# sdrobert/pydrobert-speech

Hardware: AMD Instinct MI355X
Metric: frames/s (whole node) + HBM-roofline %, 40-mel fbank 16kHz 25/10ms (higher is better)
Workload: dtype f32

## Files before the change

pydrobert-speech_amd/csrc/fft_inlane.h:

```cpp
#pragma once
#include <hip/hip_runtime.h>

#include <type_traits>

#include "twiddle_consts.h"

#define PDS_HD __host__ __device__ __forceinline__

#ifndef PDS_FMA_BUTTERFLY
#define PDS_FMA_BUTTERFLY 1
#endif

namespace pds {
namespace inl {

template <int I>
using Int = std::integral_constant<int, I>;

template <int B, int E, typename F>
PDS_HD void static_for(F &&f) {
  if constexpr (B < E) {
    f(Int<B>{});
    static_for<B + 1, E>(f);
  }
// ... 54 lines not shown
        yi[k] = si;
        yr[k + H] = fmaf(2.0f, er[k], -sr);
        yi[k + H] = fmaf(2.0f, ei[k], -si);
        return;
#endif
      }
      float tr, ti;
      mul_tw<N, k>(qr[k], qi[k], tr, ti);
      yr[k] = er[k] + tr;
      yi[k] = ei[k] + ti;
      yr[k + H] = er[k] - tr;
      yi[k + H] = ei[k] - ti;
    });
  }
};

template <int IS>
struct CFFT<1, IS> {
  static PDS_HD void run(const float *xr, const float *xi, float *yr, float *yi) {
    yr[0] = xr[0];
    yi[0] = xi[0];
  }
};

template <int IS>
struct CFFT<2, IS> {
  static PDS_HD void run(const float *xr, const float *xi, float *yr, float *yi) {
    const float ar = xr[0], ai = xi[0], br = xr[IS], bi = xi[IS];
    yr[0] = ar + br;
    yi[0] = ai + bi;
    yr[1] = ar - br;
    yi[1] = ai - bi;
  }
};

template <int IS>
struct CFFT<4, IS> {
  static PDS_HD void run(const float *xr, const float *xi, float *yr, float *yi) {
    const float ar = xr[0] + xr[2 * IS], ai = xi[0] + xi[2 * IS];
    const float br = xr[0] - xr[2 * IS], bi = xi[0] - xi[2 * IS];
    const float cr = xr[IS] + xr[3 * IS], ci = xi[IS] + xi[3 * IS];
    const float dr = xr[IS] - xr[3 * IS], di = xi[IS] - xi[3 * IS];
    yr[0] = ar + cr;
    yi[0] = ai + ci;
    yr[2] = ar - cr;
    yi[2] = ai - ci;
    yr[1] = br + di;
    yi[1] = bi - dr;
    yr[3] = br - di;
    yi[3] = bi + dr;
  }
};

template <int M>
PDS_HD void rdft_scaled(const float *a, float &even_sum, float &odd_sum, float *Ar, float *Ai) {
  constexpr int H = M / 2;
  float zr[H], zi[H];
  CFFT<H, 2>::run(a, a + 1, zr, zi);
  even_sum = zr[0];
  odd_sum = zi[0];
  if constexpr (H >= 2) {
    Ar[H / 2] = zr[H / 2];
    Ai[H / 2] = -zi[H / 2];
  }
  static_for<1, H / 2>([&](auto kk) {
    constexpr int k = decltype(kk)::value;
    const float sr = zr[k] + zr[H - k], si = zi[k] - zi[H - k];
    const float dr = zr[k] - zr[H - k], di = zi[k] + zi[H - k];
    constexpr float wr = Tw<M, k>::re, wi = Tw<M, k>::im;
#if PDS_FMA_BUTTERFLY
    const float ar = fmaf(wr, di, fmaf(wi, dr, sr));
    const float ai = fmaf(wi, di, fmaf(-wr, dr, si));
    Ar[k] = ar;
    Ai[k] = ai;
    Ar[H - k] = fmaf(2.0f, sr, -ar);
    Ai[H - k] = fmaf(-2.0f, si, ai);
#else
    const float tr = wr * di + wi * dr;
    const float ti = wi * di - wr * dr;
    Ar[k] = sr + tr;
    Ai[k] = si + ti;
    Ar[H - k] = sr - tr;
    Ai[H - k] = ti - si;
#endif
  });
}

template <int M, int IS>
struct RDIT {
  static PDS_HD void run(const float *x, float &r0, float &rh, float *Ar, float *Ai) {
    constexpr int H = M / 2, Q = M / 4;
    float e0, eh, o0, oh;
    float Er[Q > 1 ? Q : 1], Ei[Q > 1 ? Q : 1], Or[Q > 1 ? Q : 1], Oi[Q > 1 ? Q : 1];
    RDIT<H, 2 * IS>::run(x, e0, eh, Er, Ei);
    RDIT<H, 2 * IS>::run(x + IS, o0, oh, Or, Oi);
    r0 = e0 + o0;
    rh = e0 - o0;
    Ar[Q] = eh;
    Ai[Q] = -oh;
    static_for<1, Q>([&](auto kk) {
      constexpr int k = decltype(kk)::value;
      constexpr float c = Tw<M, k>::re, s = Tw<M, k>::im;
      const float ar = fmaf(Or[k], c, fmaf(-s, Oi[k], Er[k]));
      const float ai = fmaf(Or[k], s, fmaf(c, Oi[k], Ei[k]));
      Ar[k] = ar;
      Ai[k] = ai;
// ... 322 lines not shown
```

pydrobert-speech_amd/csrc/pds_internal.h:

```cpp
#pragma once
#include <hip/hip_runtime.h>
#include <stdint.h>

#include <exception>
#include <new>
#include <string>

#include "../../include/pds_amd.h"

namespace pds {

void set_error(const std::string &msg);
int32_t hip_fail(hipError_t err, const char *what);

#define PDS_HIP(call)                                       \
  do {                                                      \
    hipError_t _e = (call);                                 \
    if (_e != hipSuccess) return pds::hip_fail(_e, #call);  \
  } while (0)

struct FastTables {
  int kind = 0;
  int n1 = 0, n2 = 0;
  int rows = 0;
  int num_cus = 0;
  float *d_window = nullptr;
  float *d_twiddle = nullptr;
  float *d_tw_special = nullptr;
  float *d_win_half = nullptr;
  float *d_tw_seed = nullptr;
  float *d_ell_w = nullptr;
  int32_t *d_ell_meta = nullptr;
  int32_t *d_ell_len = nullptr;
  int32_t *d_ell_woff = nullptr;
  int ell_wfloats = 0, ell_slots = 0;
  float *d_seg_w = nullptr;
  int32_t *d_seg_meta = nullptr;
  int seg_rounds = 0, seg_len = 0, seg_wfloats = 0, seg_meta_ints = 0;
  float *d_rs_w = nullptr;
  int32_t *d_rs_meta = nullptr;
  int rs_rounds = 0, rs_len = 0, rs_wfloats = 0;
  float *d_rsn_w = nullptr;
  int32_t *d_rsn_meta = nullptr;
  int rsn_rounds = 0, rsn_len = 0, rsn_wfloats = 0;
  int rs_eslot = -1;
  float *d_ms_w = nullptr;
  int32_t *d_ms_meta = nullptr;
  int ms_rounds = 0, ms_len = 0, ms_wfloats = 0, ms_meta_ints = 0, ms_slots = 0;
  long ms_reads = 0;
  int walk = 0;
  long rs_reads = 0, rs_cost = 0, ell_reads = 0, seg_reads = 0;
  float *d_mf_tab = nullptr;
  int mf_rows = 0;
};

}

struct pds_stft_plan {
  pds_stft_desc d;
  int device = 0;
  int num_bins = 0;
  float *d_window_f32 = nullptr;
  double *d_window_f64 = nullptr;
  int32_t *d_row_ptr = nullptr;
  int32_t *d_col = nullptr;
  float *d_val_f32 = nullptr;
  double *d_val_f64 = nullptr;
  float2 *d_tw_f32 = nullptr;
  double2 *d_tw_f64 = nullptr;
  pds::FastTables fast;
};

namespace pds {
struct SiFftTables {
  int blocks = 0;
  bool big = false;
  float2 *d_spectra = nullptr;
  float2 *d_twiddle = nullptr;
  float2 *d_twiddle2k = nullptr;
  int num_cus = 0;
// ... 112 lines not shown
```

pydrobert-speech_amd/csrc/stft_fast.hip:

```cpp
#include "stft_wave_launch.h"

namespace pds {

#if PDS_STAMPS
unsigned long long *g_stamp_buf = nullptr;
extern "C" __attribute__((visibility("default"))) void pds_debug_set_stamp_buffer(unsigned long long *d_buf) {
  g_stamp_buf = d_buf;
}
#endif

extern "C" __attribute__((visibility("default"))) int32_t pds_build_experiments(void) { return PDS_EXPERIMENTS ? 1 : 0; }

bool fast_has_f64in(const pds_stft_plan *plan) { return plan->fast.kind && fast_f64in_kind(plan->fast.kind); }

bool fast_has_fused_cmvn(const pds_stft_plan *plan) {
  const FastTables &ft = plan->fast;
  return ft.kind && ft.n2 == 16 && ((ft.n1 == 64 && ft.walk != 0) || (ft.n1 == 32 && (ft.walk == 1 || ft.walk == 3)));
}

bool fast_has_fused_deltas(const pds_stft_plan *plan) {
  const FastTables &ft = plan->fast;
  return ft.kind && fast_deltas_kind(ft.kind) && ft.rsn_rounds >= 1 && ft.rsn_rounds <= 2 &&
         (!plan->d.include_energy || ft.rs_eslot >= 0);
}
// ... 43 lines not shown
#include "stft_geoms.def"
#endif
#undef PDS_GEOM
  set_error("stft_batch: no fused kernel for this plan");
  return PDS_ERR_INVALID;
}

int32_t fast_tables_create(pds_stft_plan *plan, const double *window, const int32_t *row_ptr,
                           const int32_t *col, const double *val) {
  FastTables &ft = plan->fast;
  ft.kind = 0;
  const pds_stft_desc &d = plan->d;
  int n1 = 0, n2 = 0;
  switch (d.dft_size) {
    case 128: n1 = 16; n2 = 8; break;
    case 256: n1 = 32; n2 = 8; break;
    case 512: n1 = 32; n2 = 16; break;
    case 1024: {
      const char *geom = PDS_EXPERIMENTS ? std::getenv("PDS_N1024_GEOM") : nullptr;
      const bool wide = geom && std::strcmp(geom, "32x32") == 0;
      n1 = wide ? 32 : 64;
      n2 = wide ? 32 : 16;
      break;
    }
    case 2048: n1 = 64; n2 = 32; break;
    case 4096: n1 = 64; n2 = 64; break;
    case 160: n1 = 20; n2 = 8; break;
    case 200: n1 = 25; n2 = 8; break;
    case 240: n1 = 30; n2 = 8; break;
    case 320: n1 = 20; n2 = 16; break;
    case 400: n1 = 25; n2 = 16; break;
    case 480: n1 = 30; n2 = 16; break;
    case 640: n1 = 20; n2 = 32; break;
    case 800: n1 = 25; n2 = 32; break;
    case 960: n1 = 30; n2 = 32; break;
    default: return PDS_OK;
  }
  const bool pow2 = (n1 & (n1 - 1)) == 0;
  if (!pow2 && d.frame_length != d.dft_size) return PDS_OK;
  const char *off = std::getenv("PDS_STFT_GENERIC");
  if (off && off[0] == '1') return PDS_OK;
  if (d.frame_length > d.dft_size || d.frame_length <= d.dft_size / 2) return PDS_OK;
  if (d.frame_shift >= (1 << 22)) return PDS_OK;
  if (d.use_log && !((float)d.log_floor >= 1.17549435e-38f)) return PDS_OK;
  if (d.num_filts > 32767) return PDS_OK;
  const int N = d.dft_size, H1 = n1 / 2, cols = (n1 - 1) / 2 + 1;
  std::vector<float> win((size_t)n1 * n2, 0.0f);
  for (int r = 0; r < n2; ++r)
    for (int k = 0; k < n1; ++k) {
      const int idx = n2 * k + r;
      if (idx < d.frame_length) win[(size_t)r * n1 + k] = (float)window[idx];
    }
  std::vector<float> tw((size_t)n2 * cols * 2, 0.0f);
  for (int r = 0; r < n2; ++r)
    for (int k1 = 1; k1 < cols; ++k1) {
      const double ang = -2.0 * M_PI * (double)((r * k1) % N) / (double)N;
      const double scale = (!pow2 || PDS_RDFT_DIT) ? 1.0 : (2 * k1 == H1) ? 1.0 : 0.5;
      tw[((size_t)r * cols + k1) * 2 + 0] = (float)(scale * std::cos(ang));
      tw[((size_t)r * cols + k1) * 2 + 1] = (float)(scale * std::sin(ang));
    }
  std::vector<int32_t> order(d.num_filts);
  for (int f = 0; f < d.num_filts; ++f) order[f] = f;
  auto span = [&](int f) {
    return row_ptr[f + 1] > row_ptr[f] ? col[row_ptr[f + 1] - 1] - (col[row_ptr[f]] & ~3) + 1 : 0;
  };
  std::stable_sort(order.begin(), order.end(), [&](int x, int y) { return span(x) > span(y); });
  const int slots = (d.num_filts + n2 - 1) / n2;
  const int pstr = ((N / 2 + 2 + 15) / 32) * 32 + 16;
  std::vector<int32_t> ell_meta((size_t)std::max(slots, 1) * n2, 0), ell_len(std::max(slots, USLOTS), 0),
      ell_woff(std::max(slots, USLOTS), 0);
  std::vector<float> ell_w;
  for (int sl = 0; sl < slots; ++sl) {
    int longest = 8;
    std::vector<int> first(n2, 0);
    for (int j = 0; j < n2 && sl * n2 + j < d.num_filts; ++j) {
      const int f = order[sl * n2 + j];
      if (row_ptr[f + 1] == row_ptr[f]) continue;
      first[j] = col[row_ptr[f]] & ~3;
      longest = std::max(longest, (span(f) + 7) / 8 * 8);
    }
    {
      std::vector<int> lanes;
      for (int j = 0; j < n2 && sl * n2 + j < d.num_filts; ++j)
        if (span(order[sl * n2 + j]) > 0) lanes.push_back(j);
      std::stable_sort(lanes.begin(), lanes.end(), [&](int x, int y) {
        return span(order[sl * n2 + x]) > span(order[sl * n2 + y]);
      });
      std::vector<std::vector<int>> taken(16);
      for (int j : lanes) {
        const int slack = std::min((longest - span(order[sl * n2 + j])) / 4, first[j] / 4);
        int best_shift = 0, best_cost = 1 << 30;
        for (int sh = 0; sh <= slack; ++sh) {
          const int q = first[j] / 4 - sh;
          int cost = 0;
          for (int other : taken[q % 16]) cost += other != q;
          if (cost < best_cost) {
            best_cost = cost;
            best_shift = sh;
          }
        }
        first[j] -= 4 * best_shift;
        taken[(first[j] / 4) % 16].push_back(first[j] / 4);
      }
    }
    ell_len[sl] = longest;
    ell_woff[sl] = (int32_t)ell_w.size();
// ... 98 lines not shown
      ft.rs_eslot = -1;
      if (rc == PDS_OK && fast_deltas_kind(N) && build_rseg(d.num_filts, row_ptr, col, val, N / 2 + 1, area_floats / 4, 2, rn, true)) {
        ft.rsn_rounds = rn.rounds;
        ft.rsn_len = rn.seg_len;
        ft.rsn_wfloats = (int)rn.w.size();
        for (size_t at = 0; at < rn.meta.size() && ft.rs_eslot < 0; ++at)
          if ((rn.meta[at] >> 16) == 0) ft.rs_eslot = (int)at;
        rc = upload(&ft.d_rsn_w, rn.w.data(), rn.w.size());
        if (rc == PDS_OK) rc = upload(&ft.d_rsn_meta, rn.meta.data(), rn.meta.size());
      }
      if (rc == PDS_OK) rc = upload(&ft.d_rs_w, rs.w.data(), rs.w.size());
      if (rc == PDS_OK) rc = upload(&ft.d_rs_meta, rs.meta.data(), rs.meta.size());
    }
  }
  if (n2 == 16 && pow2 && rc == PDS_OK && dense_bank) {
    MsegTables ms;
    const int area_floats = wave_area_floats(n1, n2);
    const int max_slots = (area_floats - 4 * pstr) / 16;
    if (build_mseg(d.num_filts, row_ptr, col, val, pstr, max_slots, ms)) {
      ft.ms_rounds = ms.rounds;
      ft.ms_slots = ms.slots;
      ft.ms_len = ms.seg_len;
      ft.ms_wfloats = (int)ms.w.size();
      ft.ms_meta_ints = (int)ms.meta.size();
      ft.ms_reads = ms.reads_per_lane();
      rc = upload(&ft.d_ms_w, ms.w.data(), ms.w.size());
      if (rc == PDS_OK) rc = upload(&ft.d_ms_meta, ms.meta.data(), ms.meta.size());
    }
  }
  {
    const char *force = std::getenv("PDS_STFT_WALK");
    ft.walk = ft.seg_rounds > 0 ? 1 : 0;
    const bool ms_stands_in = ft.walk == 0 && dense_bank && ft.ms_rounds > 0 && N >= PDS_MSEG_MIN_N;
    const long other = ft.walk == 1 ? ft.seg_reads : ms_stands_in ? dense_reads : ft.ell_reads;
    if (ft.rs_rounds > 0 && 10 * ft.rs_reads <= 7 * other) ft.walk = 2;
    if (force && std::strcmp(force, "ell") == 0) ft.walk = 0;
    if (force && std::strcmp(force, "seg") == 0) ft.walk = ft.seg_rounds > 0 ? 1 : 0;
    if (force && std::strcmp(force, "rseg") == 0) ft.walk = ft.rs_rounds > 0 ? 2 : ft.walk;
    if ((ft.walk == 1 || (ft.walk == 0 && ms_stands_in)) && ft.ms_rounds > 0 && N >= PDS_MSEG_MIN_N && !force) ft.walk = 3;
    if (force && std::strcmp(force, "mseg") == 0 && ft.ms_rounds > 0) ft.walk = 3;
    if (std::getenv("PDS_DEBUG_PLAN"))
      std::fprintf(stderr,
                   "pds plan N=%d filters=%d: ell slots %d reads %ld | seg rounds %d len %d reads %ld | rseg rounds %d "
                   "len %d reads %ld cost %ld | mseg rounds %d len %d reads %ld -> walk %d\n",
                   N, d.num_filts, ft.ell_slots, ft.ell_reads, ft.seg_rounds, ft.seg_len, ft.seg_reads, ft.rs_rounds,
                   ft.rs_len, ft.rs_reads, ft.rs_cost, ft.ms_rounds, ft.ms_len, ft.ms_reads, ft.walk);
  }
  if (rc == PDS_OK) rc = upload(&ft.d_ell_w, ell_w.data(), ell_w.size());
  if (rc == PDS_OK) rc = upload(&ft.d_ell_meta, ell_meta.data(), ell_meta.size());
  if (rc == PDS_OK) rc = upload(&ft.d_ell_len, ell_len.data(), ell_len.size());
  if (rc == PDS_OK) rc = upload(&ft.d_ell_woff, ell_woff.data(), ell_woff.size());
  if (rc == PDS_OK) rc = upload(&ft.d_window, win.data(), win.size());
  if (rc == PDS_OK) rc = upload(&ft.d_twiddle, tw.data(), tw.size());
  if (((n1 == 32 || n1 == 64) && n2 == 16) || lean_geometry(n1, n2)) {
    std::vector<float> wh(win), seed((size_t)n2 * 6);
    for (float &v : wh) v *= PDS_RDFT_DIT ? 1.0f : 0.5f;
    const int mult[3] = {1, 4, n1 / 4};
    for (int r = 0; r < n2; ++r)
      for (int j = 0; j < 3; ++j) {
        const double ang = -2.0 * M_PI * (double)((r * mult[j]) % N) / (double)N;
        seed[((size_t)r * 3 + j) * 2 + 0] = (float)std::cos(ang);
        seed[((size_t)r * 3 + j) * 2 + 1] = (float)std::sin(ang);
      }
    if (rc == PDS_OK) rc = upload(&ft.d_win_half, wh.data(), wh.size());
    if (rc == PDS_OK) rc = upload(&ft.d_tw_seed, seed.data(), seed.size());
  }
  std::vector<float> tws((size_t)n2 * 2);
  for (int r = 0; r < n2; ++r) {
    const double ang = -2.0 * M_PI * (double)r / (double)(2 * n2);
    tws[2 * r] = (float)std::cos(ang);
    tws[2 * r + 1] = (float)std::sin(ang);
  }
  if (rc == PDS_OK) rc = upload(&ft.d_tw_special, tws.data(), tws.size());
  {
    const char *front = PDS_EXPERIMENTS ? std::getenv("PDS_STFT_FRONT") : nullptr;
    const int rows = (d.frame_length + n2 - 1) / n2;
    int bucket = 0;
    for (int b : {20, 25, 28, 30, 32})
      if (!bucket && rows <= b) bucket = b;
    MfmaFrontTables mt;
    if (rc == PDS_OK && n1 == 32 && n2 == 16 && bucket && front && std::strcmp(front, "mfma") == 0 &&
        build_mfma_front(n1, bucket, d.frame_length, window, mt)) {
      std::vector<float> image;
      image.reserve(mt.words());
      image.insert(image.end(), mt.win.begin(), mt.win.end());
      for (int32_t v : mt.off) {
        float f;
        std::memcpy(&f, &v, sizeof f);
        image.push_back(f);
      }
      image.insert(image.end(), mt.emask.begin(), mt.emask.end());
      image.insert(image.end(), mt.a_re.begin(), mt.a_re.end());
      image.insert(image.end(), mt.a_im.begin(), mt.a_im.end());
      image.insert(image.end(), mt.tw.begin(), mt.tw.end());
      rc = upload(&ft.d_mf_tab, image.data(), image.size());
      ft.mf_rows = bucket;
    }
  }
  if (rc != PDS_OK) return rc;
  hipDeviceProp_t prop;
  PDS_HIP(hipGetDeviceProperties(&prop, plan->device));
  ft.num_cus = prop.multiProcessorCount;
  ft.n1 = n1;
  ft.n2 = n2;
  ft.rows = (d.frame_length + n2 - 1) / n2;
  ft.kind = d.dft_size;
  return PDS_OK;
}

void fast_tables_destroy(pds_stft_plan *plan) {
  FastTables &ft = plan->fast;
  (void)hipFree(ft.d_window);
  (void)hipFree(ft.d_twiddle);
  (void)hipFree(ft.d_tw_special);
  (void)hipFree(ft.d_win_half);
  (void)hipFree(ft.d_tw_seed);
  (void)hipFree(ft.d_mf_tab);
  (void)hipFree(ft.d_rs_w);
  (void)hipFree(ft.d_ms_w);
  (void)hipFree(ft.d_ms_meta);
  (void)hipFree(ft.d_rsn_w);
  (void)hipFree(ft.d_rsn_meta);
  (void)hipFree(ft.d_rs_meta);
  (void)hipFree(ft.d_seg_w);
  (void)hipFree(ft.d_seg_meta);
  (void)hipFree(ft.d_ell_w);
  (void)hipFree(ft.d_ell_meta);
  (void)hipFree(ft.d_ell_len);
  (void)hipFree(ft.d_ell_woff);
  ft = FastTables();
}

}
```

pydrobert-speech_amd/csrc/stft_switches.h:

```cpp
#pragma once
namespace pds {

#ifndef PDS_PRIO_PACK
#define PDS_PRIO_PACK 0x103212
#endif
#if PDS_PRIO_PACK == 0xffffff
#define PDS_PHASE(i) __builtin_amdgcn_sched_barrier(0)
#else
#define PDS_PHASE(i) do { if (PDS_PRIO_PACK >= 0) __builtin_amdgcn_s_setprio(((PDS_PRIO_PACK) >> (4 * (i))) & 3); } while (0)
#endif
#ifndef PDS_ABLATE
#define PDS_ABLATE 0
#endif
#ifndef PDS_STAMPS
#define PDS_STAMPS 0
#endif
#if PDS_STAMPS
extern unsigned long long *g_stamp_buf;
#define PDS_STAMP(i, drain)                                               \
  do {                                                                    \
    if (PDS_STAMPS == 2) break;                                           \
    __builtin_amdgcn_sched_barrier(0);                                    \
    if (drain) asm volatile("s_waitcnt vmcnt(0)" ::: "memory");           \
    const unsigned long long now_ = __builtin_readcyclecounter();         \
    st_acc[i] += now_ - st_prev;                                          \
    st_prev = now_;                                                       \
    __builtin_amdgcn_sched_barrier(0);                                    \
  } while (0)
#else
#define PDS_STAMP(i, drain) do { } while (0)
#endif
#ifndef PDS_SEG_DEEP_N
#define PDS_SEG_DEEP_N 1024
#endif
#ifndef PDS_ELL_DEEP_N
#define PDS_ELL_DEEP_N 4096
#endif
#ifndef PDS_MSEG_MIN_N
#define PDS_MSEG_MIN_N 1024
#endif
#ifndef PDS_PAIR_SPLIT
#define PDS_PAIR_SPLIT 1
#endif
#ifndef PDS_N4096_MINW
#define PDS_N4096_MINW 2
#endif
#ifndef PDS_FAST_PROLOGUE
#define PDS_FAST_PROLOGUE 1
#endif
#ifndef PDS_MSEG_RED4
#define PDS_MSEG_RED4 1
#endif
#ifndef PDS_FILTER_UNROLL
#define PDS_FILTER_UNROLL 2
#endif
#ifndef PDS_EXPERIMENTS
#define PDS_EXPERIMENTS 0
#endif
#ifndef PDS_RDFT_DIT
#define PDS_RDFT_DIT (!PDS_EXPERIMENTS)
#endif
#ifndef PDS_WINDOW_CONTRACT
#define PDS_WINDOW_CONTRACT 0
#endif
#ifndef PDS_PACKED_LDS
#define PDS_PACKED_LDS 0
#endif
#ifndef PDS_WALK_DPP_FMAC
#define PDS_WALK_DPP_FMAC 1
#endif
#ifndef PDS_PREEMPH_DPP
#define PDS_PREEMPH_DPP 1
#endif
#ifndef PDS_DYN
#define PDS_DYN 0
#endif
#ifndef PDS_PF_TW
#define PDS_PF_TW 1
#endif
#ifndef PDS_LEAN_1024
#define PDS_LEAN_1024 1
#endif
#ifndef PDS_DLT_CHAIN
#define PDS_DLT_CHAIN 0
#endif
#ifndef PDS_PF_WIN
#define PDS_PF_WIN 0
#endif
#ifndef PDS_PF_PLACE
#define PDS_PF_PLACE 1
#endif
#ifndef PDS_PF_WINAT
// ... 19 lines not shown
```

pydrobert-speech_amd/csrc/stft_wave_kernel.h:

```cpp
#pragma once
#include <algorithm>
#include <atomic>
#include <cmath>
#include <cstdio>
#include <cstdlib>
#include <cstring>
#include <type_traits>
#include <vector>

#include "fft_inlane.h"
#include "mfma_front.h"
#include "rseg_tables.h"
#include "mseg_tables.h"
#include "pds_internal.h"

#include "stft_switches.h"

namespace pds {

__device__ __forceinline__ void keep_alive(float v) { asm volatile("" ::"v"(v)); }

struct FastParams {
  const void *sig;
  const int64_t *offsets, *lengths, *nframes, *row_off;
  void *out;
  int64_t out_stride;
  const float *win_lane;
  const float2 *tw_lane;
  const float2 *tw_special;
  const float *win_half;
  const float2 *tw_seed;
  const float *ell_w;
  const int32_t *ell_meta;
  const int32_t *ell_len;
  const int32_t *ell_woff;
  int ell_wfloats, ell_slots, ell_meta_pad, ell_meta_ints;
  int seg_rounds, seg_len, num_filts;
  int L, S, pad_left, include_energy, use_power, use_log;
  float log_floor, inv_L, preemph;
  double preemph_d;
  int chunks_per_utt, num_utts;
  int waves;
  int area_f;
  unsigned waves_rcp;
  int lds_ticket_off;
  int dyn;
  const float *mf_tab;
  unsigned long long *stamps;
  const int64_t *chunk_prefix;
  double *stat_part;
  int stat_c, stat_cs;
  int lds_stat_off;
  int dl_inner;
  int dl_order;
  int dl_debug;
  int dl_eslot;
  float dl_f1[5], dl_f2[9];
  int step_utts, step_chunks;
};

__device__ __forceinline__ float mul_legacy(float x, float y) {
  float z;
  asm("v_mul_legacy_f32 %0, %1, %2" : "=v"(z) : "v"(x), "v"(y));
  return z;
}

template <int N1>
__device__ __forceinline__ float window_mul(int n1, float x, float w) {
#if PDS_WINDOW_CONTRACT
  return n1 < N1 / 2 ? x * w : mul_legacy(x, w);
#else
  return mul_legacy(x, w);
#endif
}

template <int M>
__device__ __forceinline__ float dpp_row_shr_keep(float old, float src) {
  return __int_as_float(__builtin_amdgcn_update_dpp(__float_as_int(old), __float_as_int(src),
                                                    0x110 + M, 0xf, 0xf, false));
}

__device__ __forceinline__ float fast_log(float x) {
  return __builtin_amdgcn_logf(x) * 0.69314718055994530942f;
}

__device__ __forceinline__ float floor_log(float v, float floor) {
  return fast_log(__builtin_elementwise_maximum(v, floor));
}

typedef int Int4 __attribute__((ext_vector_type(4)));
template <typename T>
__device__ __forceinline__ T load_const(const T *ptr) {
  typedef const T __attribute__((address_space(4))) *const_ptr;
  return *(const_ptr)(uintptr_t)ptr;
}

template <int CTRL>
__device__ __forceinline__ float dpp_add(float x) {
  return x + __int_as_float(__builtin_amdgcn_update_dpp(0, __float_as_int(x), CTRL, 0xf, 0xf, false));
}

__device__ __forceinline__ void wave_sync() {
  __builtin_amdgcn_fence(__ATOMIC_RELEASE, "wavefront");
  __builtin_amdgcn_wave_barrier();
  __builtin_amdgcn_fence(__ATOMIC_ACQUIRE, "wavefront");
}

#ifndef PDS_TWOPASS
#define PDS_TWOPASS 1
#endif
#ifndef PDS_LEAN_2048
#define PDS_LEAN_2048 1
#endif
constexpr bool lean_geometry(int n1, int n2) { return PDS_LEAN_2048 && n1 == 64 && n2 == 32; }
constexpr int wave_area_floats(int n1, int n2) {
  const int cols = (n1 - 1) / 2 + 1, groups = 64 / n2, one_pass = groups * cols * (n2 + 2) * 2;
  return (PDS_TWOPASS && n1 == 64 && n2 == 16) ? 2688 : lean_geometry(n1, n2) ? groups * cols * (n2 + 4) : one_pass;
}
constexpr int win_table_stride(int rows) { return ((rows + 3) & ~3) % 8 == 4 ? ((rows + 3) & ~3) : ((rows + 3) & ~3) + 4; }

template <int N1, int N2, int NROWS>
struct WaveGeom {
  static constexpr int N = N1 * N2;
  static constexpr int NREG = (N1 - 1) / 2;
  static constexpr int COLS = NREG + 1;
  static constexpr int CPL = (COLS + N2 - 1) / N2;
  static constexpr bool FULL = COLS % N2 == 0;
  static constexpr bool DIST = N2 >= 16;
  static constexpr int GROUPS = 64 / N2;
  static constexpr int NB = N / 2 + 1;
  static constexpr int RS = N2 + 2;
  static constexpr bool TWOPASS = PDS_TWOPASS && N1 == 64 && N2 == 16;
  static constexpr bool LEAN = lean_geometry(N1, N2);
  static constexpr int RSF = N2 + 4;
  static constexpr int XROWS = TWOPASS ? N2 : COLS;
  static constexpr int EXCH_F2 = wave_area_floats(N1, N2) / 2;
  static_assert(LEAN ? GROUPS * XROWS * RSF <= EXCH_F2 * 2 : GROUPS * XROWS * RS <= EXCH_F2, "the exchange must fit the wave's area");
  static_assert(!LEAN || (CPL == 1 && N2 >= 32), "lean form: one column per lane");
  static constexpr int PSTR = ((NB + 1 + 15) / 32) * 32 + 16;
  static_assert(GROUPS * PSTR <= EXCH_F2 * 2, "P must fit over the exchange area");
  static constexpr int XMIN_F = LEAN ? GROUPS * XROWS * RSF : GROUPS * XROWS * RS * 2;
  static constexpr int GCH = XMIN_F / 64 < NROWS ? XMIN_F / 64 : NROWS;
  static_assert(N % 2 == 0 && CPL >= 1 && N2 <= 64 && (RS * 8) % 16 == 0, "geometry");
  static_assert(inl::is_pow2(N1) ? (FULL || N2 == 2 * COLS) : 600 % N1 == 0,
                "in-lane DFT sizes: 2^k, or a divisor of 600");
  static_assert(NROWS <= N1 && NROWS > 0, "rows");
};

constexpr int USLOTS = 4;

typedef float f32x4 __attribute__((ext_vector_type(4)));

template <int N1, int N2, int NROWS, int MAXWAVES, int MINW, bool ELL_LDS, bool PRE, int SEG = 0, int MF = 0,
          bool RSG = false, typename TIN = float, typename TOUT = float, int DLT = 0, bool STR = false, bool PF = false>
__global__ __launch_bounds__(MAXWAVES * 64, MINW) void stft_wave_kernel(const FastParams p) {
  static_assert(!PF || (DLT == 0 && !STR && MF == 0 && !PRE && std::is_same<TIN, float>::value && (N1 == 32 || N1 == 64) && N2 == 16),
                "prefetch: 16-lane power-of-two geometries, float32 samples, round-robin scheduling");
  constexpr bool STRETCH = DLT > 0 || STR;
  static_assert(!(STR && DLT > 0), "stretch scheduling is part of the fused-deltas launches already");
  static_assert(DLT == 0 || (DLT == 2 && N2 == 16 && RSG && std::is_same<TOUT, float>::value && MF == 0),
                "fused deltas: row-segment walk, float32 features");
  static_assert(MF == 0 || std::is_same<TIN, float>::value, "matrix-pipe front end: float32 samples");
  static_assert(std::is_same<TIN, float>::value || std::is_same<TIN, double>::value || std::is_same<TIN, int16_t>::value, "samples: float32, float64 or int16");
  using G = WaveGeom<N1, N2, NROWS>;
  constexpr int N = G::N, COLS = G::COLS, NREG = G::NREG, RS = G::RS, NB = G::NB, PSTR = G::PSTR;
  constexpr int MSLOTS = 2 * MF + 1;
  static_assert(MF == 0 || (N2 == 16 && N1 == 32 && MF == mfma_front_steps(NROWS)), "matrix-pipe front end: 32 x 16");
  static_assert(MF == 0 || 4 * MSLOTS * 64 <= G::EXCH_F2 * 2, "edge-frame gather reuses the exchange area");
  constexpr int NBP = (NB + 3) / 4 * 4;
  static_assert(!RSG || (G::GROUPS == 4 && ELL_LDS && !SEG && (NBP + 1) * 4 <= G::EXCH_F2 * 2),
                "row-segment walk: four frames per wave, tables in LDS");
  extern __shared__ __attribute__((aligned(16))) float smem[];
  const int lane = threadIdx.x & 63;
  const int wave = __builtin_amdgcn_readfirstlane(threadIdx.x >> 6);
  const int g = lane / N2, r = lane % N2;
  constexpr bool F64S = std::is_same<TIN, double>::value;
  constexpr bool PAIR = F64S && N2 == 16 && MF == 0;
  const int rho = PAIR ? ((r & 7) * 2 + (r >> 3)) : r;
  constexpr int LOADSPAN = PAIR ? (NROWS + 1) / 2 * 32 : NROWS * N2;
  [[maybe_unused]] const unsigned long long st_entry = PDS_STAMPS ? __builtin_readcyclecounter() : 0;
  float *wbase = smem + wave * p.area_f;
  [[maybe_unused]] double *wstat = reinterpret_cast<double *>(smem + p.lds_stat_off) + wave * (2 * p.stat_cs);
  constexpr bool STATS = STR && G::GROUPS == 4 && (SEG != 0 || (RSG && MINW <= 2));
  [[maybe_unused]] const bool stats_on = STATS && p.stat_part != nullptr;
  [[maybe_unused]] auto stat_add4 = [&](const int col, const float (&v)[4], const int nf) {
    double t1 = 0.0, t2 = 0.0;
#pragma unroll
    for (int q = 0; q < 4; ++q)
      if (q < nf) {
        const double d = (double)v[q];
        t1 += d;
        t2 = fma(d, d, t2);
      }
    wstat[col] += t1;
    wstat[p.stat_cs + col] += t2;
  };
  float2 *exch = reinterpret_cast<float2 *>(wbase) + g * G::XROWS * RS;
  [[maybe_unused]] float *xf = wbase + g * (G::XROWS * G::RSF);
  float *Pg = wbase + g * PSTR;
  const int nthreads = p.waves * 64;
  float2 *sw_lds = reinterpret_cast<float2 *>(smem + p.waves * p.area_f);
  int *meta_lds = reinterpret_cast<int *>(sw_lds + N2);
  float *ellw_lds = reinterpret_cast<float *>(meta_lds + p.ell_meta_pad);
  constexpr bool TWCHAIN = (PF && PDS_PF_TW == 1) || (PAIR && (N1 == 32 || N1 == 64)) || (PDS_DLT_CHAIN && DLT > 0 && N1 == 32 && N2 == 16) || G::LEAN ||
                           (N1 == 64 && N2 == 16 && (SEG == 2 || PDS_LEAN_1024));
  constexpr bool WINLDS = PF && PDS_PF_WIN == 1;
  constexpr bool WINUSE = G::LEAN || (N1 == 64 && N2 == 16 && (SEG == 2 || PDS_LEAN_1024));
  constexpr int WSTR = win_table_stride(NROWS);
  [[maybe_unused]] float *win_lds = ellw_lds + (ELL_LDS ? p.ell_wfloats : 0);
  if constexpr (WINLDS || WINUSE) {
    const float *wsrc = TWCHAIN ? p.win_half : p.win_lane;
    for (int i = threadIdx.x; i < N2 * WSTR; i += p.waves * 64) {
      const int rr = i / WSTR, k = i - rr * WSTR;
      win_lds[i] = k < NROWS ? wsrc[rr * N1 + k] : 0.0f;
    }
  }
  if (threadIdx.x < N2) sw_lds[threadIdx.x] = p.tw_special[threadIdx.x];
  constexpr bool DYN = PDS_DYN && !STRETCH && !PF;
  [[maybe_unused]] int *ticket_lds = reinterpret_cast<int *>(smem + p.lds_ticket_off);
  if constexpr (DYN) {
    if (threadIdx.x == 0) *ticket_lds = p.waves;
  }
  if constexpr (STR && G::GROUPS == 4 && (SEG != 0 || (RSG && MINW <= 2))) {
    if (p.stat_part) {
      double *z = reinterpret_cast<double *>(smem + p.lds_stat_off);
      for (int i = threadIdx.x; i < p.waves * 2 * p.stat_cs; i += p.waves * 64) z[i] = 0.0;
    }
  }
  if constexpr (RSG) {
    int4 *rec_lds = reinterpret_cast<int4 *>(meta_lds);
    for (int i = threadIdx.x; i < p.seg_rounds * 64; i += nthreads) {
      const int m = p.ell_meta[i], f = (m >> 16) - 1;
      rec_lds[i] = make_int4((m & 0x3fff) * 16, __float_as_int((m & (1 << 14)) ? 1.0f : 0.0f),
                             __float_as_int((m & (1 << 15)) ? 1.0f : 0.0f),
                             f >= 0 ? ((p.include_energy ? 1 : 0) + f) * (int)sizeof(TOUT) : -1);
    }
  } else {
    for (int i = threadIdx.x; i < p.ell_meta_pad; i += nthreads)
      meta_lds[i] = i < p.ell_meta_ints ? p.ell_meta[i] : 0;
  }
#if PDS_FAST_PROLOGUE
  static_assert((G::EXCH_F2 * 2) % 4 == 0, "wave areas are zeroed 16 bytes at a time");
  if constexpr (ELL_LDS) {
    const float4 *src4 = reinterpret_cast<const float4 *>(p.ell_w);
    float4 *dst4 = reinterpret_cast<float4 *>(ellw_lds);
    for (int i = threadIdx.x; i < (p.ell_wfloats >> 2); i += nthreads) dst4[i] = src4[i];
  }
  {
    float4 *z4 = reinterpret_cast<float4 *>(smem);
    for (int i = threadIdx.x; i < p.waves * (p.area_f / 4); i += nthreads) z4[i] = make_float4(0.0f, 0.0f, 0.0f, 0.0f);
  }
#else
  if constexpr (ELL_LDS)
    for (int i = threadIdx.x; i < p.ell_wfloats; i += nthreads) ellw_lds[i] = p.ell_w[i];
  for (int i = threadIdx.x; i < p.waves * p.area_f; i += nthreads) smem[i] = 0.0f;
#endif
  __syncthreads();

  [[maybe_unused]] float win[(MF || WINLDS || WINUSE) ? 1 : NROWS];
  [[maybe_unused]] float twr[(MF || TWCHAIN) ? 1 : COLS], twi[(MF || TWCHAIN) ? 1 : COLS];
  [[maybe_unused]] float sd[6] = {0.0f, 0.0f, 0.0f, 0.0f, 0.0f, 0.0f};
  [[maybe_unused]] float mwin[MSLOTS], mare[MF + 1], maim[MF + 1], mtwr[4], mtwi[4];
  [[maybe_unused]] unsigned moff[MSLOTS];
  if constexpr (MF > 0) {
    const float *tab = p.mf_tab;
#pragma unroll
    for (int sl = 0; sl < MSLOTS; ++sl) {
      mwin[sl] = tab[sl * 64 + lane];
      moff[sl] = (unsigned)reinterpret_cast<const int *>(tab)[(MSLOTS + sl) * 64 + lane] * 4u;
    }
#pragma unroll
    for (int t = 0; t <= MF; ++t) {
      mare[t] = tab[(3 * MSLOTS + t) * 64 + lane];
      maim[t] = tab[(3 * MSLOTS + MF + 1 + t) * 64 + lane];
    }
#pragma unroll
    for (int v = 0; v < 4; ++v) {
      const float2 t = reinterpret_cast<const float2 *>(tab + (3 * MSLOTS + 2 * (MF + 1)) * 64)[v * 64 + lane];
      mtwr[v] = t.x;
      mtwi[v] = t.y;
    }
  } else {
    if constexpr (!WINLDS && !WINUSE) {
      const float *wsrc = TWCHAIN ? p.win_half : p.win_lane;
#pragma unroll
      for (int n1 = 0; n1 < NROWS; ++n1) win[n1] = wsrc[rho * N1 + n1];
    }
    if constexpr (TWCHAIN) {
#pragma unroll
      for (int j = 0; j < 3; ++j) {
        const float2 t = p.tw_seed[rho * 3 + j];
        sd[2 * j] = t.x;
        sd[2 * j + 1] = t.y;
      }
    } else {
#pragma unroll
      for (int k1 = 1; k1 <= NREG; ++k1) {
        const float2 t = p.tw_lane[rho * COLS + k1];
        twr[k1] = t.x;
        twi[k1] = t.y;
      }
    }
  }
  [[maybe_unused]] float pfv[PF ? NROWS : 1];
  [[maybe_unused]] float wl[WINLDS ? NROWS : 1];
  [[maybe_unused]] auto read_window = [&]() {
    if constexpr (WINLDS) {
      const float4 *w4 = reinterpret_cast<const float4 *>(win_lds + rho * WSTR);
#pragma unroll
      for (int j = 0; j < (NROWS + 3) / 4; ++j) {
        const float4 w = w4[j];
        const float wv[4] = {w.x, w.y, w.z, w.w};
#pragma unroll
        for (int u = 0; u < 4; ++u)
          if (4 * j + u < NROWS) wl[4 * j + u] = wv[u];
      }
    }
  };
  read_window();
  [[maybe_unused]] bool pf_ready = false;
  [[maybe_unused]] const int pf_lane = __mul24(g, p.S) + r;
  const int L = p.L, S = p.S;
  const bool use_power = p.use_power != 0;
  const int col0 = p.include_energy ? 1 : 0;

  int b = 0;
  int wg = blockIdx.x;
#ifndef PDS_NO_XCD_MAP
  if ((gridDim.x & 7) == 0) wg = (wg & 7) * (gridDim.x >> 3) + (wg >> 3);
#endif
  int chunk = wg * p.waves + wave;
  if constexpr (!STRETCH) {
    while (chunk >= p.chunks_per_utt && b < p.num_utts) {
      chunk -= p.chunks_per_utt;
      ++b;
    }
  }
  [[maybe_unused]] int rnd = 0, rb = 0, rc = wg * p.waves;
  if constexpr (DYN) {
    while (rc >= p.chunks_per_utt && rb < p.num_utts) {
      rc -= p.chunks_per_utt;
      ++rb;
    }
  }
  [[maybe_unused]] auto take_ticket = [&](const int t) {
    const int jn = (int)__umulhi((unsigned)t, p.waves_rcp), o = t - jn * p.waves;
    while (rnd < jn && rb < p.num_utts) {
      rc += p.step_chunks;
      rb += p.step_utts;
      if (rc >= p.chunks_per_utt) {
        rc -= p.chunks_per_utt;
        ++rb;
      }
      ++rnd;
    }
// ... 560 lines not shown
        for (int n1 = 0; n1 < NROWS; ++n1) a[n1] = window_mul<N1>(n1, a[n1], wl[n1]);
      } else if constexpr (WINUSE) {
        const float4 *w4 = reinterpret_cast<const float4 *>(win_lds + rho * WSTR);
#pragma unroll
        for (int j = 0; j < (NROWS + 3) / 4; ++j) {
          const float4 w = w4[j];
          const float wv[4] = {w.x, w.y, w.z, w.w};
#pragma unroll
          for (int u = 0; u < 4; ++u)
            if (4 * j + u < NROWS) a[4 * j + u] = window_mul<N1>(4 * j + u, a[4 * j + u], wv[u]);
        }
      } else {
#pragma unroll
        for (int n1 = 0; n1 < NROWS; ++n1) a[n1] = window_mul<N1>(n1, a[n1], win[n1]);
      }
      if constexpr (PF) fetch_next_record();
#pragma unroll
      for (int n1 = NROWS; n1 < N1; ++n1) a[n1] = 0.0f;

      if constexpr (PDS_ABLATE & 2) {
        even_sum = a[0];
        odd_sum = a[1];
#pragma unroll
        for (int k = 0; k < COLS; ++k) {
          Ar[k] = a[2 * k];
          Ai[k] = a[2 * k + 1];
        }
      } else if constexpr (inl::is_pow2(N1)) {
#if PDS_RDFT_DIT
        inl::rdft_dit<N1>(a, even_sum, odd_sum, Ar, Ai);
#else
        inl::rdft_scaled<N1>(a, even_sum, odd_sum, Ar, Ai);
#endif
      } else {
        inl::rdft_direct<N1>(a, even_sum, odd_sum, Ar, Ai);
      }

      PDS_PHASE(1);
      if constexpr (G::LEAN) {
        const int slot = (rho & 1) ? N2 + (rho & 3) : (rho >> 1);
        xf[slot] = even_sum;
        xf[(rho & 1) ? N2 + (rho & 3) : N2 / 2 + (rho >> 1)] = odd_sum;
      } else {
        float *row0 = reinterpret_cast<float *>(exch);
        row0[rho] = even_sum;
        row0[N2 + rho] = odd_sum;
      }
      [[maybe_unused]] float ctr[TWCHAIN ? COLS : 1], cti[TWCHAIN ? COLS : 1];
      if constexpr (TWCHAIN) {
#pragma unroll
        for (int j = 0; j < 6; ++j) asm volatile("" : "+v"(sd[j]));
        inl::twiddle_chain<NREG, !PDS_RDFT_DIT>(sd[0], sd[1], sd[2], sd[3], sd[4], sd[5], ctr, cti);
      }
#pragma unroll
      for (int k1 = 1; k1 <= NREG; ++k1) {
        const float wr_ = TWCHAIN ? ctr[TWCHAIN ? k1 : 0] : twr[TWCHAIN ? 0 : k1];
        const float wi_ = TWCHAIN ? cti[TWCHAIN ? k1 : 0] : twi[TWCHAIN ? 0 : k1];
        float2 v;
        v.x = Ar[k1] * wr_ - Ai[k1] * wi_;
        v.y = Ar[k1] * wi_ + Ai[k1] * wr_;
        if constexpr ((PDS_ABLATE & 4) != 0) {
          Ar[k1] = v.x;
          Ai[k1] = v.y;
        } else if (G::TWOPASS && k1 >= N2) {
          Ar[k1] = v.x;
          Ai[k1] = v.y;
        } else if constexpr (G::LEAN) {
          xf[k1 * G::RSF + rho] = v.x;
          Ai[k1] = v.y;
        } else {
          exch[k1 * RS + rho] = v;
        }
      }
    }
    PDS_STAMP(2, 0);
    wave_sync();

    float pw[G::CPL][N2 + 1];
    float sp0 = 0.0f, sp1 = 0.0f;
    constexpr bool PSPLIT = PDS_PAIR_SPLIT && N2 == 2 * COLS && (N2 == 64 || N2 == 32);
    constexpr int PH = N2 / 2, PQ = N2 / 4;
    [[maybe_unused]] const int ph = r / (N2 / 2), pc = r % (N2 / 2);
    if constexpr (PSPLIT) {
      static_assert(!PSPLIT || (G::CPL == 1 && COLS == PH), "pair split: the columns fill half the frame's lanes");
      const float4 *row = reinterpret_cast<const float4 *>(exch + pc * RS);
      float zr[PH], zi[PH], Hr[PH], Hi[PH];
#pragma unroll
      for (int j = 0; j < PH; ++j) {
        const float4 v = row[j];
        zr[j] = ph ? v.z : v.x;
        zi[j] = ph ? v.w : v.y;
      }
      PDS_PHASE(5);
      inl::CFFT<PH, 1>::run(zr, zi, Hr, Hi);
      PDS_PHASE(2);
      inl::static_for<0, PQ>([&](auto k_) {
        constexpr int k = decltype(k_)::value;
        float ar, br, ai, bi;
        if constexpr (N2 == 64) {
          const auto sr_ = __builtin_amdgcn_permlane32_swap(__float_as_uint(Hr[k]), __float_as_uint(Hr[k + PQ]), false, false);
          const auto si_ = __builtin_amdgcn_permlane32_swap(__float_as_uint(Hi[k]), __float_as_uint(Hi[k + PQ]), false, false);
          ar = __uint_as_float(sr_[0]), br = __uint_as_float(sr_[1]);
          ai = __uint_as_float(si_[0]), bi = __uint_as_float(si_[1]);
        } else {
          const auto sr_ = __builtin_amdgcn_permlane16_swap(__float_as_uint(Hr[k]), __float_as_uint(Hr[k + PQ]), false, false);
          const auto si_ = __builtin_amdgcn_permlane16_swap(__float_as_uint(Hi[k]), __float_as_uint(Hi[k + PQ]), false, false);
          ar = __uint_as_float(sr_[0]), br = __uint_as_float(sr_[1]);
          ai = __uint_as_float(si_[0]), bi = __uint_as_float(si_[1]);
        }
        float ur, ui;
// ... 36 lines not shown
      }
      const float4 *row = reinterpret_cast<const float4 *>(exch + (G::TWOPASS ? r : kk) * RS);
      float zr[N2], zi[N2], Yr[N2], Yi[N2];
      if constexpr (G::LEAN) {
        const float4 *rowf = reinterpret_cast<const float4 *>(xf + r * G::RSF);
#pragma unroll
        for (int j = 0; j < N2 / 4; ++j) {
          const float4 v = rowf[j];
          zr[4 * j] = v.x, zr[4 * j + 1] = v.y, zr[4 * j + 2] = v.z, zr[4 * j + 3] = v.w;
        }
        wave_sync();
        {
          const int slot = (rho & 1) ? (rho >> 1) : N2 + (rho & 3);
          xf[slot] = even_sum;
          xf[(rho & 1) ? N2 / 2 + (rho >> 1) : N2 + (rho & 3)] = odd_sum;
        }
#pragma unroll
        for (int k1 = 1; k1 <= NREG; ++k1) xf[k1 * G::RSF + rho] = Ai[k1];
        wave_sync();
#pragma unroll
        for (int j = 0; j < N2 / 4; ++j) {
          const float4 v = rowf[j];
          zi[4 * j] = v.x, zi[4 * j + 1] = v.y, zi[4 * j + 2] = v.z, zi[4 * j + 3] = v.w;
        }
      } else
#pragma unroll
      for (int j = 0; j < N2 / 2; ++j) {
        float4 v;
        if constexpr (PDS_ABLATE & 4) {
          v = make_float4(Ar[(2 * j) % COLS], Ai[(2 * j) % COLS], Ar[(2 * j + 1) % COLS], Ai[(2 * j + 1) % COLS]);
        } else {
          v = row[j];
        }
        zr[2 * j] = v.x;
        zi[2 * j] = v.y;
        zr[2 * j + 1] = v.z;
        zi[2 * j + 1] = v.w;
      }
      if constexpr (PF && PDS_PF_PLACE == 0) {
        PDS_PHASE(5);
#if PDS_PF_ILV > 0
        __builtin_amdgcn_sched_group_barrier(0x100, N2 / 2, 0);
#endif
        if (q == 0) issue_prefetch();
      }
      if constexpr (PDS_ABLATE & 8) {
#pragma unroll
        for (int k2 = 0; k2 < N2; ++k2) {
          Yr[k2] = zr[k2];
          Yi[k2] = zi[k2];
        }
      } else {
        if constexpr (!(PF && PDS_PF_PLACE == 0)) PDS_PHASE(5);
        inl::CFFT<N2, 1>::run(zr, zi, Yr, Yi);
        if (q + 1 < G::CPL) {
          PDS_PHASE(1);
        } else {
          PDS_PHASE(2);
        }
      }
#pragma unroll
      for (int k2 = 0; k2 < N2; ++k2) pw[q][k2] = Yr[k2] * Yr[k2] + Yi[k2] * Yi[k2];
      pw[q][N2] = 0.0f;
      if constexpr (!G::DIST) {
        if (q == 0 && r == 0)
          inl::rdft_finish_power<2 * N2>(Yr, Yi, [&](auto mm, float re, float im) {
            pw[q][decltype(mm)::value] = re * re + im * im;
          });
      } else if (q == 0) {
        float ar, ai, br, bi;
        if constexpr (N2 == 16 && !PDS_PACKED_LDS) {
          ar = Yr[0], ai = Yi[0], br = Yr[0], bi = Yi[0];
          inl::static_for<1, N2 / 2 + 1>([&](auto mm) {
            constexpr int m = decltype(mm)::value;
            ar = dpp_row_shr_keep<m>(ar, Yr[m]);
            ai = dpp_row_shr_keep<m>(ai, Yi[m]);
            br = dpp_row_shr_keep<m>(br, Yr[N2 - m]);
            bi = dpp_row_shr_keep<m>(bi, Yi[N2 - m]);
          });
        } else {
          float2 *hand = G::LEAN ? reinterpret_cast<float2 *>(xf) : exch;
          if (r == 0) {
            if constexpr (N2 % 2 == 0) {
              float4 *hand4 = reinterpret_cast<float4 *>(hand);
#pragma unroll
              for (int k2 = 0; k2 < N2; k2 += 2) hand4[k2 / 2] = make_float4(Yr[k2], Yi[k2], Yr[k2 + 1], Yi[k2 + 1]);
            } else {
#pragma unroll
              for (int k2 = 0; k2 < N2; ++k2) hand[k2] = make_float2(Yr[k2], Yi[k2]);
            }
          }
          wave_sync();
          const float2 ya = hand[r], yb = hand[(N2 - r) & (N2 - 1)];
          ar = ya.x, ai = ya.y, br = yb.x, bi = yb.y;
        }
        const float sr = ar + br, si = ai - bi;
        const float dr = ar - br, di = ai + bi;
        const float tr = sw.x * di + sw.y * dr;
        const float ti = sw.y * di - sw.x * dr;
        const float xr = sr + tr, xi = si + ti;
        const float yr = sr - tr, yi = ti - si;
        sp0 = (TWCHAIN && !PDS_RDFT_DIT ? 1.0f : 0.25f) * (xr * xr + xi * xi);
        sp1 = (TWCHAIN && !PDS_RDFT_DIT ? 1.0f : 0.25f) * (yr * yr + yi * yi);
      }
    }
    if (!use_power) {
#pragma unroll
// ... 497 lines not shown
```

pydrobert-speech_amd/csrc/stft_wave_launch.h:

```cpp
#pragma once
#include "stft_wave_kernel.h"

namespace pds {


constexpr bool fast_f64in_kind(int n) { return n == 256 || n == 512 || n == 1024 || n == 2048; }

constexpr bool fast_deltas_kind(int n) { return n == 512 || n == 1024; }


template <int N1, int N2, int NROWS, int MINW>
int32_t launch_wave(const pds_stft_plan *plan, const BatchArgs &a) {
  using G = WaveGeom<N1, N2, NROWS>;
#ifndef PDS_DLT_MINW
#define PDS_DLT_MINW 3
#endif
  constexpr int DMINW = (N1 == 64 && N2 == 16) ? 2 : MINW > PDS_DLT_MINW ? PDS_DLT_MINW : MINW;
  constexpr int CU_WAVES_STFT = 4 * MINW;
  constexpr int F64_MINW = (N1 == 64 && N2 == 16) ? 2 : MINW, F64_WAVES = 4 * F64_MINW;
  const int CU_WAVES = a.dl_K > 0 ? 4 * DMINW : a.in_f64 ? F64_WAVES : CU_WAVES_STFT;
  const FastTables &ft = plan->fast;
  FastParams p;
  p.sig = a.d_signal;
  p.offsets = a.d_offsets;
  p.lengths = a.d_lengths;
  p.nframes = a.d_nframes;
  p.row_off = a.d_row_off;
  p.out = a.d_out;
  p.out_stride = a.out_stride;
  p.win_lane = ft.d_window;
  p.tw_lane = (const float2 *)ft.d_twiddle;
  p.tw_special = (const float2 *)ft.d_tw_special;
  constexpr bool LEAN_ALL = G::LEAN || (PDS_LEAN_1024 && N1 == 64 && N2 == 16);
  p.win_half = LEAN_ALL ? ft.d_win_half : nullptr;
  p.tw_seed = LEAN_ALL ? (const float2 *)ft.d_tw_seed : nullptr;
  p.ell_w = ft.d_ell_w;
  p.ell_meta = ft.d_ell_meta;
  p.ell_len = ft.d_ell_len;
  p.ell_woff = ft.d_ell_woff;
  p.ell_wfloats = ft.ell_wfloats;
  p.ell_slots = ft.ell_slots;
  p.L = plan->d.frame_length;
  p.S = plan->d.frame_shift;
  p.pad_left = a.pad_left;
  p.include_energy = plan->d.include_energy;
  p.use_power = plan->d.use_power;
  p.use_log = plan->d.use_log;
  p.log_floor = (float)plan->d.log_floor;
  p.inv_L = 1.0f / (float)plan->d.frame_length;
  p.num_utts = a.B;
  const int64_t chunks = (a.max_frames + G::GROUPS - 1) / G::GROUPS;
  if (chunks * a.B > 0x7fffffff || chunks > 0x3fffffff || a.out_stride * G::GROUPS > (a.out_f64 ? 0x0fffffff : 0x1fffffff) ||
      a.max_frames * plan->d.frame_shift > 0x7fffffff) {
    set_error("stft_batch: too many frame chunks in one call");
    return PDS_ERR_INVALID;
  }
  p.chunks_per_utt = (int)chunks;
  const size_t lds_cu = 160 * 1024;
  const size_t per_wave = (size_t)G::EXCH_F2 * 8;
  const int stat_c = a.d_stat_part ? plan->d.num_filts + (plan->d.include_energy ? 1 : 0) : 0;
  const int stat_cs = (stat_c + 3) & ~3;
  const size_t stat_pw = (size_t)2 * stat_cs * 8;
  int shapes[4][2] = {{CU_WAVES / 2, 2}, {CU_WAVES, 1}, {CU_WAVES * 3 / 4, 1}, {CU_WAVES * 5 / 8, 1}};
#ifdef PDS_ONE_WG
  shapes[0][0] = CU_WAVES, shapes[0][1] = 1;
#endif
  if (CU_WAVES % 8 != 0) {
    shapes[0][0] = CU_WAVES, shapes[0][1] = 1;
    shapes[1][0] = CU_WAVES * 2 / 3, shapes[1][1] = 1;
    shapes[2][0] = CU_WAVES / 3, shapes[2][1] = 1;
    shapes[3][0] = CU_WAVES / 3, shapes[3][1] = 1;
  }
  constexpr int CU_WAVES_K = CU_WAVES_STFT;
  int waves = CU_WAVES / 2, wgs_per_cu = 2;
  size_t area_bytes = per_wave;
  bool in_lds = false;
  p.seg_rounds = 0;
  p.seg_len = 0;
  p.num_filts = plan->d.num_filts;
  const bool pre = a.preemph != 0.0;
  int walk = 0;
  const bool dl = a.dl_K > 0 && ft.rsn_rounds > 0;
  constexpr bool PFG = (N1 == 32 || N1 == 64) && N2 == 16;
  const char *pf_env = std::getenv("PDS_STFT_PF");
// ... 287 lines not shown
```

Baseline: 4.043 billion.

## Fold four-step FFT inter-stage twiddles into the column transform butterflies

Adds a twiddled column FFT (CFFT_TW) that applies the per-column inter-stage twiddle factors inside its first radix-4 butterflies as FMAs, instead of a separate complex multiply pass before the LDS exchange. A new per-column twiddle table is built on the host and uploaded, and each lane preloads CPL*N2 twiddles into registers. Radix-2 stages use the 2a-s FMA trick to save adds. The goal is fewer ALU ops in the FFT, at the cost of more registers held for twiddles, which may lower occupancy or cause spills for the 512-point geometry.

Result: no change. 4.023 billion (-0.5%).

```diff
diff --git a/pydrobert-speech_amd/csrc/fft_inlane.h b/pydrobert-speech_amd/csrc/fft_inlane.h
--- a/pydrobert-speech_amd/csrc/fft_inlane.h
+++ b/pydrobert-speech_amd/csrc/fft_inlane.h
@@ -130,6 +130,76 @@
   }
 };
 
+template <int N, int IS, int OFF>
+struct CFFT_TWR {
+  static PDS_HD void run(const float *xr, const float *xi, const float *tr, const float *ti, float *yr, float *yi) {
+    constexpr int H = N / 2;
+    float er[H], ei[H], qr[H], qi[H];
+    CFFT_TWR<H, 2 * IS, OFF>::run(xr, xi, tr, ti, er, ei);
+    CFFT_TWR<H, 2 * IS, OFF + IS>::run(xr, xi, tr, ti, qr, qi);
+    static_for<0, H>([&](auto kk) {
+      constexpr int k = decltype(kk)::value;
+      if constexpr (k != 0 && 4 * k != N && 8 * k != N && 8 * k != 3 * N) {
+        constexpr float c = Tw<N, k>::re, s = Tw<N, k>::im;
+        const float sr = fmaf(qr[k], c, fmaf(-s, qi[k], er[k]));
+        const float si = fmaf(qr[k], s, fmaf(c, qi[k], ei[k]));
+        yr[k] = sr;
+        yi[k] = si;
+        yr[k + H] = fmaf(2.0f, er[k], -sr);
+        yi[k + H] = fmaf(2.0f, ei[k], -si);
+      } else {
+        float ur, ui;
+        mul_tw<N, k>(qr[k], qi[k], ur, ui);
+        yr[k] = er[k] + ur;
+        yi[k] = ei[k] + ui;
+        yr[k + H] = er[k] - ur;
+        yi[k + H] = ei[k] - ui;
+      }
+    });
+  }
+};
+
+template <int IS, int OFF>
+struct CFFT_TWR<4, IS, OFF> {
+  template <int J, int K>
+  static PDS_HD void pair(const float *xr, const float *xi, const float *tr, const float *ti, float &sr, float &si,
+                          float &dr, float &di) {
+    float pr, pi;
+    if constexpr (J == 0) {
+      pr = xr[0];
+      pi = xi[0];
+    } else {
+      pr = fmaf(xr[J], tr[J], -(xi[J] * ti[J]));
+      pi = fmaf(xr[J], ti[J], xi[J] * tr[J]);
+    }
+    sr = fmaf(xr[K], tr[K], fmaf(-ti[K], xi[K], pr));
+    si = fmaf(xr[K], ti[K], fmaf(tr[K], xi[K], pi));
+    dr = fmaf(2.0f, pr, -sr);
+    di = fmaf(2.0f, pi, -si);
+  }
+  static PDS_HD void run(const float *xr, const float *xi, const float *tr, const float *ti, float *yr, float *yi) {
+    float ar, ai, br, bi, cr, ci, dr, di;
+    pair<OFF, OFF + 2 * IS>(xr, xi, tr, ti, ar, ai, br, bi);
+    pair<OFF + IS, OFF + 3 * IS>(xr, xi, tr, ti, cr, ci, dr, di);
+    yr[0] = ar + cr;
+    yi[0] = ai + ci;
+    yr[2] = ar - cr;
+    yi[2] = ai - ci;
+    yr[1] = br + di;
+    yi[1] = bi - dr;
+    yr[3] = br - di;
+    yi[3] = bi + dr;
+  }
+};
+
+template <int N>
+struct CFFT_TW {
+  static_assert(N >= 4 && (N & (N - 1)) == 0, "twiddled column transform: a power of two from 4 up");
+  static PDS_HD void run(const float *xr, const float *xi, const float *tr, const float *ti, float *yr, float *yi) {
+    CFFT_TWR<N, 1, 0>::run(xr, xi, tr, ti, yr, yi);
+  }
+};
+
 template <int M>
 PDS_HD void rdft_scaled(const float *a, float &even_sum, float &odd_sum, float *Ar, float *Ai) {
   constexpr int H = M / 2;
diff --git a/pydrobert-speech_amd/csrc/pds_internal.h b/pydrobert-speech_amd/csrc/pds_internal.h
--- a/pydrobert-speech_amd/csrc/pds_internal.h
+++ b/pydrobert-speech_amd/csrc/pds_internal.h
@@ -26,6 +26,7 @@
   int num_cus = 0;
   float *d_window = nullptr;
   float *d_twiddle = nullptr;
+  float *d_tw_col = nullptr;
   float *d_tw_special = nullptr;
   float *d_win_half = nullptr;
   float *d_tw_seed = nullptr;
diff --git a/pydrobert-speech_amd/csrc/stft_fast.hip b/pydrobert-speech_amd/csrc/stft_fast.hip
--- a/pydrobert-speech_amd/csrc/stft_fast.hip
+++ b/pydrobert-speech_amd/csrc/stft_fast.hip
@@ -119,6 +119,16 @@
       if (idx < d.frame_length) win[(size_t)r * n1 + k] = (float)window[idx];
     }
   std::vector<float> tw((size_t)n2 * cols * 2, 0.0f);
+  std::vector<float> twc;
+  if (tw_fold_geometry(n1, n2)) {
+    twc.resize((size_t)cols * n2 * 2);
+    for (int c = 0; c < cols; ++c)
+      for (int n = 0; n < n2; ++n) {
+        const double ang = -2.0 * M_PI * (double)((c * n) % N) / (double)N;
+        twc[((size_t)c * n2 + n) * 2 + 0] = (float)std::cos(ang);
+        twc[((size_t)c * n2 + n) * 2 + 1] = (float)std::sin(ang);
+      }
+  }
   for (int r = 0; r < n2; ++r)
     for (int k1 = 1; k1 < cols; ++k1) {
       const double ang = -2.0 * M_PI * (double)((r * k1) % N) / (double)N;
@@ -323,6 +333,7 @@
   if (rc == PDS_OK) rc = upload(&ft.d_ell_woff, ell_woff.data(), ell_woff.size());
   if (rc == PDS_OK) rc = upload(&ft.d_window, win.data(), win.size());
   if (rc == PDS_OK) rc = upload(&ft.d_twiddle, tw.data(), tw.size());
+  if (rc == PDS_OK && !twc.empty()) rc = upload(&ft.d_tw_col, twc.data(), twc.size());
   if (((n1 == 32 || n1 == 64) && n2 == 16) || lean_geometry(n1, n2)) {
     std::vector<float> wh(win), seed((size_t)n2 * 6);
     for (float &v : wh) v *= PDS_RDFT_DIT ? 1.0f : 0.5f;
@@ -383,6 +394,7 @@
   FastTables &ft = plan->fast;
   (void)hipFree(ft.d_window);
   (void)hipFree(ft.d_twiddle);
+  (void)hipFree(ft.d_tw_col);
   (void)hipFree(ft.d_tw_special);
   (void)hipFree(ft.d_win_half);
   (void)hipFree(ft.d_tw_seed);
diff --git a/pydrobert-speech_amd/csrc/stft_switches.h b/pydrobert-speech_amd/csrc/stft_switches.h
--- a/pydrobert-speech_amd/csrc/stft_switches.h
+++ b/pydrobert-speech_amd/csrc/stft_switches.h
@@ -38,6 +38,9 @@
 #endif
 #ifndef PDS_MSEG_MIN_N
 #define PDS_MSEG_MIN_N 1024
+#endif
+#ifndef PDS_TW_FOLD
+#define PDS_TW_FOLD 1
 #endif
 #ifndef PDS_PAIR_SPLIT
 #define PDS_PAIR_SPLIT 1
diff --git a/pydrobert-speech_amd/csrc/stft_wave_kernel.h b/pydrobert-speech_amd/csrc/stft_wave_kernel.h
--- a/pydrobert-speech_amd/csrc/stft_wave_kernel.h
+++ b/pydrobert-speech_amd/csrc/stft_wave_kernel.h
@@ -27,6 +27,7 @@
   int64_t out_stride;
   const float *win_lane;
   const float2 *tw_lane;
+  const float2 *tw_col;
   const float2 *tw_special;
   const float *win_half;
   const float2 *tw_seed;
@@ -113,6 +114,10 @@
 #define PDS_LEAN_2048 1
 #endif
 constexpr bool lean_geometry(int n1, int n2) { return PDS_LEAN_2048 && n1 == 64 && n2 == 32; }
+constexpr bool tw_fold_geometry(int n1, int n2) {
+  return PDS_TW_FOLD && PDS_RDFT_DIT && PDS_ABLATE == 0 && inl::is_pow2(n1) && (n1 / 2) % n2 == 0 && !lean_geometry(n1, n2) &&
+         !(PDS_TWOPASS && n1 == 64 && n2 == 16);
+}
 constexpr int wave_area_floats(int n1, int n2) {
   const int cols = (n1 - 1) / 2 + 1, groups = 64 / n2, one_pass = groups * cols * (n2 + 2) * 2;
   return (PDS_TWOPASS && n1 == 64 && n2 == 16) ? 2688 : lean_geometry(n1, n2) ? groups * cols * (n2 + 4) : one_pass;
@@ -204,6 +209,7 @@
   float *ellw_lds = reinterpret_cast<float *>(meta_lds + p.ell_meta_pad);
   constexpr bool TWCHAIN = (PF && PDS_PF_TW == 1) || (PAIR && (N1 == 32 || N1 == 64)) || (PDS_DLT_CHAIN && DLT > 0 && N1 == 32 && N2 == 16) || G::LEAN ||
                            (N1 == 64 && N2 == 16 && (SEG == 2 || PDS_LEAN_1024));
+  constexpr bool TWFOLD = tw_fold_geometry(N1, N2) && MF == 0 && !TWCHAIN && SEG == 0;
   constexpr bool WINLDS = PF && PDS_PF_WIN == 1;
   constexpr bool WINUSE = G::LEAN || (N1 == 64 && N2 == 16 && (SEG == 2 || PDS_LEAN_1024));
   constexpr int WSTR = win_table_stride(NROWS);
@@ -258,7 +264,8 @@
   __syncthreads();
 
   [[maybe_unused]] float win[(MF || WINLDS || WINUSE) ? 1 : NROWS];
-  [[maybe_unused]] float twr[(MF || TWCHAIN) ? 1 : COLS], twi[(MF || TWCHAIN) ? 1 : COLS];
+  constexpr int NTW = (MF || TWCHAIN) ? 1 : TWFOLD ? G::CPL * N2 : COLS;
+  [[maybe_unused]] float twr[NTW], twi[NTW];
   [[maybe_unused]] float sd[6] = {0.0f, 0.0f, 0.0f, 0.0f, 0.0f, 0.0f};
   [[maybe_unused]] float mwin[MSLOTS], mare[MF + 1], maim[MF + 1], mtwr[4], mtwi[4];
   [[maybe_unused]] unsigned moff[MSLOTS];
@@ -293,6 +300,15 @@
         sd[2 * j] = t.x;
         sd[2 * j + 1] = t.y;
       }
+    } else if constexpr (TWFOLD) {
+#pragma unroll
+      for (int q = 0; q < G::CPL; ++q)
+#pragma unroll
+        for (int n2 = 1; n2 < N2; ++n2) {
+          const float2 t = p.tw_col[(q * N2 + r) * N2 + n2];
+          twr[q * N2 + n2] = t.x;
+          twi[q * N2 + n2] = t.y;
+        }
     } else {
 #pragma unroll
       for (int k1 = 1; k1 <= NREG; ++k1) {
@@ -301,6 +317,10 @@
         twi[k1] = t.y;
       }
     }
+  }
+  if constexpr (TWFOLD && !WINLDS && !WINUSE) {
+#pragma unroll
+    for (int n1 = 0; n1 < NROWS; ++n1) asm volatile("" : "+v"(win[n1]));
   }
   [[maybe_unused]] float pfv[PF ? NROWS : 1];
   [[maybe_unused]] float wl[WINLDS ? NROWS : 1];
@@ -967,10 +987,14 @@
         for (int j = 0; j < 6; ++j) asm volatile("" : "+v"(sd[j]));
         inl::twiddle_chain<NREG, !PDS_RDFT_DIT>(sd[0], sd[1], sd[2], sd[3], sd[4], sd[5], ctr, cti);
       }
+      if constexpr (TWFOLD) {
+#pragma unroll
+        for (int k1 = 1; k1 <= NREG; ++k1) exch[k1 * RS + rho] = make_float2(Ar[k1], Ai[k1]);
+      } else
 #pragma unroll
       for (int k1 = 1; k1 <= NREG; ++k1) {
-        const float wr_ = TWCHAIN ? ctr[TWCHAIN ? k1 : 0] : twr[TWCHAIN ? 0 : k1];
-        const float wi_ = TWCHAIN ? cti[TWCHAIN ? k1 : 0] : twi[TWCHAIN ? 0 : k1];
+        const float wr_ = TWCHAIN ? ctr[TWCHAIN ? k1 : 0] : twr[(TWCHAIN || TWFOLD) ? 0 : k1];
+        const float wi_ = TWCHAIN ? cti[TWCHAIN ? k1 : 0] : twi[(TWCHAIN || TWFOLD) ? 0 : k1];
         float2 v;
         v.x = Ar[k1] * wr_ - Ai[k1] * wi_;
         v.y = Ar[k1] * wi_ + Ai[k1] * wr_;
@@ -1113,7 +1137,11 @@
         }
       } else {
         if constexpr (!(PF && PDS_PF_PLACE == 0)) PDS_PHASE(5);
-        inl::CFFT<N2, 1>::run(zr, zi, Yr, Yi);
+        if constexpr (TWFOLD) {
+          inl::CFFT_TW<N2>::run(zr, zi, twr + (TWFOLD ? q * N2 : 0), twi + (TWFOLD ? q * N2 : 0), Yr, Yi);
+        } else {
+          inl::CFFT<N2, 1>::run(zr, zi, Yr, Yi);
+        }
         if (q + 1 < G::CPL) {
           PDS_PHASE(1);
         } else {
diff --git a/pydrobert-speech_amd/csrc/stft_wave_launch.h b/pydrobert-speech_amd/csrc/stft_wave_launch.h
--- a/pydrobert-speech_amd/csrc/stft_wave_launch.h
+++ b/pydrobert-speech_amd/csrc/stft_wave_launch.h
@@ -30,6 +30,7 @@
   p.out_stride = a.out_stride;
   p.win_lane = ft.d_window;
   p.tw_lane = (const float2 *)ft.d_twiddle;
+  p.tw_col = (const float2 *)ft.d_tw_col;
   p.tw_special = (const float2 *)ft.d_tw_special;
   constexpr bool LEAN_ALL = G::LEAN || (PDS_LEAN_1024 && N1 == 64 && N2 == 16);
   p.win_half = LEAN_ALL ? ft.d_win_half : nullptr;
```
